# drtconway/zotmer

Hardware: AMD Instinct MI355X
Metric: Gk-mers/sec kmerize k=25 on synthetic 150bp FASTQ; achieved HBM GB/s fraction (higher is better)
Workload: dtype u64

## Files before the change

### zotmer_amd/csrc/context.hip

```cpp
#include <stdarg.h>
#include <string.h>

#include "internal.hpp"
#include <vector>

namespace zk {

int fail(zk_ctx* c, int code, const char* fmt, ...) {
    char buf[512];
    va_list ap;
    va_start(ap, fmt);
    vsnprintf(buf, sizeof buf, fmt, ap);
    va_end(ap);
    if (c) c->last_error = buf;
    return code;
}

void arena_reset(zk_ctx* c) { c->arena_off = 0; }

int arena_alloc(zk_ctx* c, uint64_t bytes, void** p) {
    const uint64_t need = (bytes + 255) & ~255ull;
    if (c->arena_off + need > c->arena_size) {
        if (c->arena_off != 0)
            return fail(c, ZK_ENOMEM, "workspace too small: %llu bytes in use, %llu more needed, %llu reserved (call zk_reserve)",
// ... 292 lines not shown
    if (what == ZK_TUNE_STREAM_PASS) {
#ifdef ZK_PHASES
        c->stream_pass = value < 0 ? 0 : value;
#else
        if (value < 0 || value > 3) return fail(c, ZK_EINVAL, "stream pass variant %d (0, 1, 2 or 3)", value);
        c->stream_pass = value;
#endif
        return ZK_OK;
    }
    if (what == ZK_TUNE_TAG_WORDS) { c->tag_words = value < 0 ? 0 : (value > 2 ? 2 : value); return ZK_OK; }
    if (what == ZK_TUNE_DEDUPE_VARIANT) { c->dedupe_variant = value < 0 ? -1 : (value & 3); return ZK_OK; }
    if (what == ZK_TUNE_KWAY) { c->kway = value < 0 ? 0 : (value > 2 ? 2 : value); return ZK_OK; }
    if (what == ZK_TUNE_TILE_SORT) { c->tile_sort = value ? 1 : 0; return ZK_OK; }
    if (what == ZK_TUNE_TAG_PASS) { c->tag_pass = value ? 1 : 0; return ZK_OK; }
    if (what == ZK_TUNE_DEDUPE_BITS) { c->dedupe_bits = value < 0 ? 0 : value; return ZK_OK; }
    if (what == ZK_TUNE_STRAND_BLOCKS) { c->strand_blocks = value < 0 ? 0 : (value > 3 ? 1 : value); return ZK_OK; }
    if (what == ZK_TUNE_DEDUPE_LIMIT) { c->dedupe_limit = value < 1 ? 1 : (value > 65536 ? 65536 : value); return ZK_OK; }
    if (what == ZK_TUNE_STREAM_RANGES) { c->stream_ranges = value < 0 ? 0 : (value > 4096 ? 4096 : value); return ZK_OK; }
    if (what == ZK_TUNE_XCD_GROUP) {
        if (value < 0 || value > 32 || (value & (value - 1))) return fail(c, ZK_EINVAL, "xcd group must be 0 or a power of two <= 32");
        c->xcd_group = value;
        return ZK_OK;
    }
    return fail(c, ZK_EINVAL, "unknown tuning knob %d", what);
}

int zk_debug_buffer(zk_ctx* c, void* d_buf) {
    if (!c) return ZK_EINVAL;
    enter(c);
    c->dbg = (u64*)d_buf;
    return ZK_OK;
// ... 99 lines not shown
```

### zotmer_amd/csrc/dedupe.hpp

```cpp
#pragma once
#include "internal.hpp"

namespace zk {

struct DedupeArgs {
    const u64* kin;
    const u32* tin;
    u64 n;
    const u64* cuts;
    u64* out;
    u64* nwords;
    int tag_bits;
    int pack;
    u32* flags;
    u32* counter;
    u64* big;
    u32* n_big;
    u32 big_cap;
    u32 chunks;
    u32* sub;
    u32* bad;
    u32* n_bad;
    u32 bad_cap;
    const u32* list;
    u32* retry;
    u32* n_retry;
    u32 limit;
    u64* dbg;
};

#ifdef ZK_PHASES
#define DD_PHASE(k) do { if (a.dbg) { const u32 now__ = (u32)__builtin_amdgcn_s_memtime(); ph[k] += now__ - tlast; tlast = now__; } } while (0)
#else
#define DD_PHASE(k) do { } while (0)
#endif

int launch_dedupe2(zk_ctx* c, const DedupeArgs& a, bool tagin, int variant, bool unsorted);

}
```

### zotmer_amd/csrc/dedupe2.hip

```cpp
#include "dedupe.hpp"
#include <type_traits>

namespace zk {

template <int BLOCK_, int BATCH_, int ITEMS_>
struct Dedupe2Smem {
    static constexpr int BLOCK = BLOCK_, BATCH = BATCH_, ITEMS = ITEMS_, TILE = BLOCK * ITEMS, NW = BLOCK / 64, ALL = 11264, SPT = ALL / BLOCK,
                         NB = 1024, SIDE = 64 + 64 * BATCH;
    static_assert(ALL % BLOCK == 0 && ALL % 8 == 0 && ITEMS % BATCH == 0 && ITEMS % 4 == 0, "whole rounds, whole quads, whole batches");
    alignas(16) u32 keys[ALL];
    alignas(16) u32 cnt[ALL / 2];
    union {
        u32 side[NW][SIDE];
        struct { u32 bc[NB]; u32 bbase[NB + 1]; } g;
    };
    u32 ticket;
    u32 nout;
};

template <int ITEMS>
struct Dedupe2Next {
    u32 chunk;
    u64 lo;
    u32 len;
    u32 tag[ITEMS];
};

template <int BLOCK, int ITEMS, bool TAGIN>
__device__ __forceinline__ void dedupe2_load(const DedupeArgs& a, u64 lo, u32 pos, u32 rem, u32 tmask, u32 (&t)[ITEMS]) {
    constexpr u32 TILE = BLOCK * ITEMS;
    u32 tid = threadIdx.x;
    asm volatile("" : "+v"(tid));
    if constexpr (TAGIN) {
// ... 11 lines not shown
            for (int i = 0; i < ITEMS; i++) {
                const u32 g = (u32)i * BLOCK + tid;
                t[i] = g < rem ? tp[g] : 0u;
            }
        }
    } else {
        const u64* kp = a.kin + lo + pos;
#pragma unroll
        for (int i = 0; i < ITEMS; i++) {
            const u32 g = (u32)i * BLOCK + tid;
            t[i] = g < rem ? (u32)kp[g] & tmask : 0u;
        }
    }
}

template <int BLOCK, int BATCH, int ITEMS_, bool TAGIN, bool UNSORTED>
__device__ __forceinline__ void dedupe2_block(const DedupeArgs& a, Dedupe2Smem<BLOCK, BATCH, ITEMS_>& sm, Dedupe2Next<ITEMS_>& st, u32 (&ph)[8], u32& tlast) {
    using S = Dedupe2Smem<BLOCK, BATCH, ITEMS_>;
    constexpr int ITEMS = S::ITEMS, TILE = S::TILE, ALL = S::ALL, SPT = S::SPT, NB = S::NB;
    constexpr u32 EMPTY = ~0u;
    constexpr u32 HS = ALL - 1;
    int tid = threadIdx.x;
    asm volatile("" : "+v"(tid));
    const int lane = tid & 63, wave = __builtin_amdgcn_readfirstlane(tid >> 6);
    const u32 chunk = st.chunk;
    const u64 lo = st.lo;
    const u32 len = st.len;
    const u32 maxc = (1u << a.pack) - 1u;
    const u32 tmask = a.tag_bits >= 32 ? ~0u : (1u << a.tag_bits) - 1u;
    auto next_block = [&](u32 t) {
        st.chunk = t; st.lo = 0; st.len = 0;
        if (t < a.chunks) {
            const u64 nlo = a.cuts[t], nhi = a.cuts[t + 1];
            st.lo = nlo;
// ... 76 lines not shown
    }
    drain(0, nside);
    DD_PHASE(1);
    const int any_bad = __syncthreads_or((int)bad);
    DD_PHASE(2);
    if (any_bad) {
        if (tid == 0) {
            a.retry[atomicAdd(a.n_retry, 1u)] = chunk;
            a.nwords[chunk] = 0;
        }
        if (a.sub && tid < 64) a.sub[(u64)chunk * 64 + tid] = 0;
        next_block(nchunk);
        return;
    }
    if constexpr (UNSORTED) {
        next_block(nchunk);
        const u16* cnt16 = reinterpret_cast<const u16*>(sm.cnt);
        u32 wn = 0;
#pragma unroll
        for (int j = 0; j < SPT; j++) wn += (u32)__popcll(__ballot(cnt16[tid + j * BLOCK] != 0));
        u32 wbase = 0;
        if (lane == 0 && wn) wbase = atomicAdd(&sm.nout, wn);
        wbase = (u32)__shfl((int)wbase, 0, 64);
        DD_PHASE(3);
        const u64 hi_part = (u64)chunk << a.tag_bits;
#pragma unroll
        for (int j = 0; j < SPT; j++) {
            const u32 c = cnt16[tid + j * BLOCK];
            const u64 bal = __ballot(c != 0);
            if (c) {
                const u64 k = hi_part | (u64)sm.keys[tid + j * BLOCK];
                if (c > maxc) {
                    const u32 at = atomicAdd(a.n_big, 1u);
                    if (at < a.big_cap) { a.big[2 * (u64)at] = k; a.big[2 * (u64)at + 1] = c; }
                    atomicOr(a.flags, 2u);
                }
                a.out[lo + wbase + popc_below(bal)] = (k << a.pack) | (u64)(c > maxc ? 0u : c);
            }
            wbase += (u32)__popcll(bal);
        }
        __syncthreads();
        if (tid == 0) a.nwords[chunk] = sm.nout;
        DD_PHASE(5);
        return;
    }
    for (int q = tid; q < NB; q += BLOCK) sm.g.bc[q] = 0;
    u32 et[SPT], ec[SPT];
    const int gb = a.tag_bits < 10 ? a.tag_bits : 10, bsh = a.tag_bits - gb;
    const u16* cnt16 = reinterpret_cast<const u16*>(sm.cnt);
#pragma unroll
    for (int j = 0; j < SPT; j++) {
        et[j] = sm.keys[tid + j * BLOCK];
        ec[j] = cnt16[tid + j * BLOCK];
    }
// ... 70 lines not shown
            const u32 i = i0 + e * BLOCK;
            if (i >= total) break;
            const u32 c = cc[e];
            const u64 k = hi_part | (u64)mine[e];
            if (c > maxc) {
                const u32 at = atomicAdd(a.n_big, 1u);
                if (at < a.big_cap) { a.big[2 * (u64)at] = k; a.big[2 * (u64)at + 1] = c; }
                atomicOr(a.flags, 2u);
            }
            a.out[lo + g0[e] + rank[e]] = (k << a.pack) | (u64)(c > maxc ? 0u : c);
        }
    }
    DD_PHASE(5);
}

template <int BLOCK, int BATCH, int ITEMS, bool TAGIN, bool UNSORTED>
__global__ __launch_bounds__(BLOCK, 2 * BLOCK / 256) void dedupe2_kernel(DedupeArgs a) {
    using S = Dedupe2Smem<BLOCK, BATCH, ITEMS>;
    __shared__ S sm;
    static_assert(sizeof(S) <= 80 * 1024, "two workgroups per CU");
    Dedupe2Next<ITEMS> st;
    if (threadIdx.x == 0) sm.ticket = atomicAdd(a.counter, 1u);
    __syncthreads();
    st.chunk = (u32)__builtin_amdgcn_readfirstlane((int)sm.ticket);
    st.lo = 0; st.len = 0;
    const u32 tmask = a.tag_bits >= 32 ? ~0u : (1u << a.tag_bits) - 1u;
    if (st.chunk < a.chunks) {
        const u64 nlo = a.cuts[st.chunk], nhi = a.cuts[st.chunk + 1];
        st.lo = nlo;
        st.len = nhi - nlo < (u64)a.limit ? (u32)(nhi - nlo) : ~0u;
    }
    if (st.len - 1u < ~0u - 1u) dedupe2_load<BLOCK, ITEMS, TAGIN>(a, st.lo, 0, st.len, tmask, st.tag);
    __syncthreads();
    u32 ph[8] = {0, 0, 0, 0, 0, 0, 0, 0};
    u32 tlast = a.dbg ? (u32)__builtin_amdgcn_s_memtime() : 0u;
    (void)tlast;
    u32 nblk = 0;
    while (st.chunk < a.chunks) {
        dedupe2_block<BLOCK, BATCH, ITEMS, TAGIN, UNSORTED>(a, sm, st, ph, tlast);
        __syncthreads();
        DD_PHASE(6);
        nblk++;
    }
    if (a.dbg && threadIdx.x == 0 && blockIdx.x < 256) {
        for (int k = 0; k < 8; k++) a.dbg[(u64)blockIdx.x * 16 + k] = ph[k];
        a.dbg[(u64)blockIdx.x * 16 + 8] = nblk;
    }
}

int launch_dedupe2(zk_ctx* c, const DedupeArgs& a, bool tagin, int variant, bool unsorted) {
    const u32 want = 2u * (u32)c->num_cus;
    const u32 grid = a.chunks < want ? a.chunks : want;
#define ZK_DD2(N, T, U) hipLaunchKernelGGL((dedupe2_kernel<512, N, 8, T, U>), dim3(grid), dim3(512), 0, c->stream, a)
#define ZK_DD2B(T, U) switch (variant & 3) { case 1: ZK_DD2(1, T, U); break; case 2: ZK_DD2(2, T, U); break; default: ZK_DD2(4, T, U); break; }
    if (unsorted) {
        if (tagin) ZK_DD2B(true, true) else ZK_DD2B(false, true)
    } else {
        if (tagin) ZK_DD2B(true, false) else ZK_DD2B(false, false)
    }
#undef ZK_DD2B
#undef ZK_DD2
    ZK_HIP(c, hipGetLastError());
    return ZK_OK;
}

}
```

### zotmer_amd/csrc/dedupe_blocks.hip

```cpp
#include "internal.hpp"
#include "dedupe.hpp"

namespace zk {

template <bool TAG32>
struct DedupeSmem {
    static constexpr int BLOCK = 1024, ITEMS = 8, TILE = BLOCK * ITEMS, NW = BLOCK / 64, ALL = TAG32 ? 12288 : 6144, SPT = ALL / BLOCK, NB = 256;
    static constexpr int SIDE_KEEP = 128, SIDE = SIDE_KEEP + 64 * ITEMS;
    typedef typename std::conditional<TAG32, u32, u64>::type E;
    E keys[ALL];
    u32 cnt[ALL];
    E side[NW][SIDE];
    u32 bc[NB];
    u32 bbase[NB + 1];
    u32 bfill[NB];
    u32 ticket;
};

__global__ void dedupe_cuts_kernel(const u64* __restrict__ k, u64 n, int tag_bits, u32 blocks, u64* __restrict__ cuts) {
    const u32 v = blockIdx.x * blockDim.x + threadIdx.x;
    if (v > blocks) return;
    u64 lo = 0, hi = n;
    while (lo < hi) {
        const u64 mid = (lo + hi) >> 1;
// ... 319 lines not shown
    }
}

int expand_tags(zk_ctx* c, const u32* tags, const u64* cuts, uint32_t blocks, int tag_bits, u64* keys_out, uint64_t first_block, uint64_t n_blocks) {
    if (n_blocks == 0) { first_block = 0; n_blocks = blocks; }
    hipLaunchKernelGGL(expand_tags_kernel, dim3(grid_cap(c, n_blocks, 16)), dim3(256), 0, c->stream, tags, cuts, (u64)first_block, (u64)n_blocks,
                       tag_bits, keys_out);
    ZK_HIP(c, hipGetLastError());
    return ZK_OK;
}

constexpr u32 DEDUPE_BIG_CAP = 1u << 16;
constexpr u32 DEDUPE_BAD_CAP = 64;

static int dedupe_lists(zk_ctx* c, const u64* keys, uint64_t n, int key_bits, int b, int pack, u64* work, uint64_t max_chunks,
                        const u32* tags, const u64* tag_cuts, bool unsorted, bool two_per_cu, DedupeArgs& a, DedupeResult* r) {
    uint64_t chunks = 1ull << b;
    if (max_chunks && chunks > max_chunks) chunks = max_chunks;
    u64 *cuts, *nwords, *incl, *big;
    if (tags) {
        if (!tag_cuts || key_bits - b > 32) return fail(c, ZK_EINTERNAL, "dedupe_pass: tags of %d bits", key_bits - b);
        cuts = const_cast<u64*>(tag_cuts);
    } else ZK_TRY(arena_alloc(c, sizeof(u64) * (chunks + 1), (void**)&cuts));
    ZK_TRY(arena_alloc(c, sizeof(u64) * chunks, (void**)&nwords));
    ZK_TRY(arena_alloc(c, sizeof(u64) * chunks, (void**)&incl));
    ZK_TRY(arena_alloc(c, sizeof(u64) * 2 * DEDUPE_BIG_CAP, (void**)&big));
    a.tag_bits = key_bits - b;
    if (!tags) hipLaunchKernelGGL(dedupe_cuts_kernel, dim3((u32)div_up(chunks + 1, 256)), dim3(256), 0, c->stream, keys, (u64)n, a.tag_bits, (u32)chunks, cuts);
    a.kin = keys; a.tin = tags; a.n = n; a.cuts = cuts; a.out = work; a.nwords = nwords; a.pack = pack;
    a.chunks = (u32)chunks;
    a.flags = (u32*)&c->d_scalars->dedupe_flags;
    a.counter = (u32*)&c->d_scalars->dedupe_counter;
    a.n_big = (u32*)&c->d_scalars->dedupe_n_big;
    a.big = big; a.big_cap = DEDUPE_BIG_CAP;
    ZK_TRY(arena_alloc(c, sizeof(u32) * DEDUPE_BAD_CAP, (void**)&a.bad));
    a.bad_cap = DEDUPE_BAD_CAP;
    a.n_bad = (u32*)&c->d_scalars->dedupe_n_bad;
    a.dbg = c->dbg ? c->dbg + 8192 : nullptr;
    unsorted = unsorted && two_per_cu;
    if (!max_chunks && !unsorted && a.tag_bits >= 14 && c->arena_size - c->arena_off > 64ull * chunks * (4 + 8 + 8) + (32ull << 20) + n / 16)
        ZK_TRY(arena_alloc(c, sizeof(u32) * 64 * chunks, (void**)&a.sub));
    ZK_HIP(c, hipMemsetAsync(&c->d_scalars->dedupe_flags, 0, ZK_SPAN(dedupe_flags, dedupe_n_bad), c->stream));
    r->cuts = cuts; r->nwords = nwords; r->incl = incl; r->big = big; r->chunks = (uint32_t)chunks; r->pack = pack; r->work = work;
    r->tag_bits = a.tag_bits; r->unsorted = unsorted;
    return ZK_OK;
}

static void launch_one_per_cu(zk_ctx* c, const DedupeArgs& d) {
    const u32 grid = d.chunks < (u32)c->num_cus ? d.chunks : (u32)c->num_cus;
    if (d.tin) hipLaunchKernelGGL((dedupe_kernel<true, true>), dim3(grid), dim3(1024), 0, c->stream, d);
    else if (d.tag_bits <= 32) hipLaunchKernelGGL((dedupe_kernel<true, false>), dim3(grid), dim3(1024), 0, c->stream, d);
    else hipLaunchKernelGGL((dedupe_kernel<false, false>), dim3(grid), dim3(1024), 0, c->stream, d);
}

static int dedupe_launch(zk_ctx* c, DedupeArgs& a, bool two_per_cu, bool unsorted) {
    prof_begin(c, ZK_PROF_RLE, (a.tin ? 4 : 8) * a.n);
    if (two_per_cu) {
        ZK_TRY(arena_alloc(c, sizeof(u32) * a.chunks, (void**)&a.retry));
        a.n_retry = (u32*)&c->d_scalars->dedupe_n_retry;
        a.limit = (u32)c->dedupe_limit;
        ZK_TRY(launch_dedupe2(c, a, a.tin != nullptr, c->dedupe_variant, unsorted));
    } else launch_one_per_cu(c, a);
    prof_end(c);
    ZK_HIP(c, hipGetLastError());
    ZK_TRY(fetch_span(c, &c->h_scalars->dedupe_flags, ZK_SPAN(dedupe_flags, dedupe_n_bad)));
    ZK_TRY(fetch(c, &c->h_scalars->dedupe_n_in, a.cuts + a.chunks));
    ZK_TRY(check_device_error(c));
    if (two_per_cu && (uint32_t)c->h_scalars->dedupe_n_retry) {
        DedupeArgs d = a;
        d.list = a.retry; d.chunks = (uint32_t)c->h_scalars->dedupe_n_retry; d.retry = nullptr; d.n_retry = nullptr;
        ZK_HIP(c, hipMemsetAsync(a.counter, 0, sizeof(u32), c->stream));
        launch_one_per_cu(c, d);
        ZK_HIP(c, hipGetLastError());
        ZK_TRY(fetch_span(c, &c->h_scalars->dedupe_flags, ZK_SPAN(dedupe_flags, dedupe_n_bad)));
        ZK_TRY(check_device_error(c));
    }
    return ZK_OK;
}

static int dedupe_bad_blocks(zk_ctx* c, const DedupeArgs& a, uint32_t n_bad, DedupeResult* r) {
    uint32_t list[DEDUPE_BAD_CAP];
    ZK_HIP(c, hipMemcpy(list, a.bad, sizeof(u32) * n_bad, hipMemcpyDeviceToHost));
    for (uint32_t i = 0; i < n_bad && !(r->flags & 1); i++) {
        u64 lohi[2];
        ZK_HIP(c, hipMemcpy(lohi, a.cuts + list[i], 2 * sizeof(u64), hipMemcpyDeviceToHost));
        const uint64_t m = lohi[1] - lohi[0];
        u64* res = nullptr;
        u64* bk = const_cast<u64*>(a.kin) + lohi[0];
        if (a.tin) {
            ZK_TRY(arena_alloc(c, 8 * m, (void**)&bk));
            ZK_TRY(expand_tags(c, a.tin, a.cuts, a.chunks, a.tag_bits, bk - lohi[0], list[i], 1));
        }
        ZK_TRY(sort_keys(c, bk, a.out + lohi[0], m, a.tag_bits, &res));
        if (res != bk) ZK_HIP(c, hipMemcpyAsync(bk, res, 8 * m, hipMemcpyDeviceToDevice, c->stream));
        uint64_t u = 0;
        bool ovf = false;
        ZK_TRY(rle(c, bk, m, a.out + lohi[0], nullptr, m, &u, a.pack, &ovf));
        if (ovf) { r->flags |= 1; break; }
        ZK_HIP(c, hipMemcpy(a.nwords + list[i], &u, sizeof(u64), hipMemcpyHostToDevice));
    }
    return ZK_OK;
}

int dedupe_pass(zk_ctx* c, const u64* keys, uint64_t n, int key_bits, int b, int pack, u64* work, uint64_t cap, DedupeResult* r,
                uint64_t* n_in, uint64_t max_chunks, const u32* tags, const u64* tag_cuts, bool unsorted) {
    *r = DedupeResult();
    if (n_in) *n_in = n;
    if (n == 0) return ZK_OK;
    if (b < 1 || b > 24 || b >= key_bits || pack < 10 || pack > 31) return fail(c, ZK_EINTERNAL, "dedupe_pass: %d block bits of %d, pack %d", b, key_bits, pack);
    if (cap < n) return fail(c, ZK_ENOSPC, "dedupe_pass: work buffer of %llu words for %llu keys", (unsigned long long)cap, (unsigned long long)n);
    DedupeArgs a = {};
    const bool two_per_cu = key_bits - b <= 32 && c->dedupe_variant >= 0;
    ZK_TRY(dedupe_lists(c, keys, n, key_bits, b, pack, work, max_chunks, tags, tag_cuts, unsorted, two_per_cu, a, r));
    ZK_TRY(dedupe_launch(c, a, two_per_cu, r->unsorted));
    r->flags = (uint32_t)c->h_scalars->dedupe_flags;
    r->n_big = (uint32_t)c->h_scalars->dedupe_n_big;
    if (r->n_big > DEDUPE_BIG_CAP) r->flags |= 1;
    const uint32_t n_bad = (uint32_t)c->h_scalars->dedupe_n_bad;
    if (n_bad && n_bad <= DEDUPE_BAD_CAP && !(r->flags & 1) && !max_chunks) {
        ZK_TRY(dedupe_bad_blocks(c, a, n_bad, r));
        a.sub = nullptr;
    } else if (n_bad > DEDUPE_BAD_CAP) r->flags |= 1;
    ZK_HIP(c, hipMemcpyAsync(r->incl, r->nwords, sizeof(u64) * r->chunks, hipMemcpyDeviceToDevice, c->stream));
    ZK_TRY(scan64_inclusive(c, r->incl, r->chunks));
    ZK_TRY(fetch(c, &c->h_scalars->dedupe_n_out, r->incl + r->chunks - 1));
    ZK_TRY(stream_sync(c));
    r->n_out = c->h_scalars->dedupe_n_out;
    prof_add_bytes(c, ZK_PROF_RLE, 8 * r->n_out);
    r->sub = a.sub;
// ... 52 lines not shown
```

### zotmer_amd/csrc/internal.hpp

```cpp
#pragma once
#include <hip/hip_runtime.h>
#include <stddef.h>
#include <stdint.h>
#include <stdio.h>
#include <string>
#include <vector>

#include "../../include/zotk.h"
#include "common.hpp"

struct zk_strand_counters { u32 n_declined, fail; };
struct zk_scalars {
    u64 rle_side;
    u64 total;
    u64 acgt[4];
    u64 n_keys;
    u64 rec_info[3];
    u64 sample_n;
    u64 dedupe_flags, dedupe_n_retry, dedupe_counter, dedupe_n_big, dedupe_n_bad;
    u64 dedupe_n_in;
    u64 dedupe_n_out;
    zk_strand_counters strand;
    u64 hist_big_n;
    u64 capture_kept;
    u64 capture_raw;
    u64 intersect_n;
    u64 checksum[3];
    u64 checksum_any[3];
    u64 stream_checksum[7];
    u64 first_descent;
    u64 ingest_cut;
    u64 sample_heads;
    u64 rle_overflow;
    u64 reduce_max;
// ... 13 lines not shown
    u64 vars[4];
    u64 links_bad;
    u64 render_bad;
    u64 render_bytes;
    u64 pileup_cursor;
    u64 pileup_long;
    u64 pulldown_vetoed;
    u64 capkmers_bad;
    u64 capkmers_total;
    u64 path_total;
    u64 place_bad;
    u64 place_slots;
    u64 seqtally[4];
};
#define ZK_SPAN(first, last) (offsetof(zk_scalars, last) + sizeof(zk_scalars::last) - offsetof(zk_scalars, first))
static_assert(sizeof(zk_scalars) == 81 * sizeof(u64), "zk_scalars: u64 words only, no padding");
static_assert(ZK_SPAN(rle_side, total) == 2 * sizeof(u64), "rle_prefix reads rle_side and total back as one range");
static_assert(ZK_SPAN(total, acgt) == 5 * sizeof(u64), "the merges read total and acgt back as one range");
static_assert(ZK_SPAN(acgt, n_keys) == 5 * sizeof(u64) && ZK_SPAN(acgt, sample_n) == 9 * sizeof(u64),
              "sort_stream reads acgt, n_keys, rec_info and sample_n back as one range");
static_assert(ZK_SPAN(rec_info, sample_n) == 4 * sizeof(u64), "sort_stream clears rec_info and sample_n as one range");
static_assert(offsetof(zk_scalars, dedupe_n_retry) == offsetof(zk_scalars, dedupe_flags) + 8 &&
              offsetof(zk_scalars, dedupe_counter) == offsetof(zk_scalars, dedupe_flags) + 16 &&
              offsetof(zk_scalars, dedupe_n_big) == offsetof(zk_scalars, dedupe_flags) + 24 &&
              ZK_SPAN(dedupe_flags, dedupe_n_bad) == 5 * sizeof(u64), "dedupe_pass clears and reads its five words as one range");

struct zk_ctx {
    int device = 0;
    hipStream_t stream = nullptr;
    bool own_stream = false;
    int num_cus = 256;
    int sort_variant = 3;
    int short_sort = 0;
    int packed_pairs = 1;
    int wide_tiles = 1;
    int early_collapse = 1;
    int side_div = 8;
    int pairs_variant = 7;
    int stream_pass = 1;
    int tag_words = 2;
// ... 112 lines not shown
int sort_pairs_mirrored(zk_ctx* c, const u64* src_k, const u32* src_v, u64* keys, u64* alt, u32* vals, u32* valt, uint64_t n, int K,
                        u64** rk, u32** rv, int lo_bit = 0);
int sort_pairs_rbits(zk_ctx* c);
struct StreamSample { int shift; uint64_t value; double max_ratio; uint64_t seen = 0, distinct = 0; bool want_distinct = false; };
struct StreamTags { bool written = false; u64* cuts = nullptr; uint32_t blocks = 0; };
struct StreamSrc { const u8* stream; uint64_t n_bytes; int K; int mode; int lo_bit; int hi_bit = 0; StreamSample* sample = nullptr;
                   StreamTags* tags = nullptr; };
int sort_stream(zk_ctx* c, const StreamSrc& src, u64* buf_a, u64* buf_b, uint64_t cap, uint64_t* n_keys,
                uint64_t acgt[4], u64** result);
int sort_rbits(zk_ctx* c);
PassPlan sort_plan_upper(zk_ctx* c, int key_bits, int lo_bit);
int sort_first_bits(zk_ctx* c, int key_bits, int lo_bit);
constexpr int MIRROR_RBITS = 9, MIRROR_RADIX = 1 << MIRROR_RBITS;
struct MirrorHist { int passes; int shift[4]; int bits[4]; u64* raw; };
int sort_keys_upper_counted(zk_ctx* c, u64* keys, u64* alt, uint64_t n, int key_bits, int lo_bit, u64* counted, u64** result);
struct DedupeResult {
    uint64_t n_out = 0;
    uint32_t flags = 0;
    uint32_t n_big = 0;
    u64 *cuts = nullptr, *nwords = nullptr, *incl = nullptr, *big = nullptr, *work = nullptr;
    u32* sub = nullptr;
    uint32_t chunks = 0;
    int pack = 0;
    int tag_bits = 0;
    bool unsorted = false;
};
int dedupe_pass(zk_ctx* c, const u64* keys, uint64_t n, int key_bits, int b, int pack, u64* work, uint64_t cap, DedupeResult* r,
                uint64_t* n_in = nullptr, uint64_t max_chunks = 0, const u32* tags = nullptr, const u64* tag_cuts = nullptr,
                bool unsorted = false);
int expand_tags(zk_ctx* c, const u32* tags, const u64* cuts, uint32_t blocks, int tag_bits, u64* keys_out, uint64_t first_block = 0, uint64_t n_blocks = 0);
int dedupe_finish(zk_ctx* c, const DedupeResult& r, u64* out_k, u32* out_c, u64* out_m = nullptr, int K = 0, int gbases = 0,
                  u64** mirror_hist = nullptr, int* mirror_group_bits = nullptr, bool packed_out = false);
int dedupe_sort_blocks(zk_ctx* c, DedupeResult& r);
int strand_blocks(zk_ctx* c, const DedupeResult& r, u64* keys_buf, uint64_t buf_words, int K, u64* out_k, u32* out_c, uint64_t cap,
                  uint64_t* n_out);
int collapse_pass(zk_ctx* c, const u64* keys, uint64_t n, int shift, int bits, int pack, u64* out, uint64_t cap, uint64_t* n_out,
                  uint64_t max_tiles = 0);
struct StreamRows { u32* rows = nullptr; u64* offs = nullptr; u32 ranges = 0, radix = 0; u32* gcodes = nullptr; u16* gvalid = nullptr;
                    u32 strands = 1;
                    bool wide = false; };
int stream_hist(zk_ctx* c, const u8* stream, uint64_t n_bytes, int K, int mode, const PassPlan& plan, u64* ghist, u32 gstride,
                u64* d_acgt, u64* d_n, u64* rec_info, u64* sample, u32 sample_cap, int sample_shift, u64 sample_value, u32* sample_n,
                void* image_room, uint64_t image_room_bytes, StreamRows* out);
struct StreamPlanes { u16* dig; int shift, bits; };
// ... 55 lines not shown
```

### zotmer_amd/csrc/pipeline.hip

```cpp
#include <string.h>

#include <vector>

#include "internal.hpp"

namespace zk {

__global__ void mirror_kernel(const u64* __restrict__ c, const u32* __restrict__ n, u64 m, int K, u64* __restrict__ r,
                              u32* __restrict__ v) {
    for (u64 i = (u64)blockIdx.x * blockDim.x + threadIdx.x; i < m; i += (u64)gridDim.x * blockDim.x) {
        r[i] = revcomp(K, c[i]);
        v[i] = n[i];
    }
}

constexpr int MIRROR_GROUP_BITS = 18;
constexpr int MIRROR_GROUP_BASES = MIRROR_GROUP_BITS / 2;

__global__ void mirror_bounds_kernel(const u64* __restrict__ c, u64 n, int K, int gbits, u64* __restrict__ start) {
    const u32 g = blockIdx.x * blockDim.x + threadIdx.x;
    if (g > (1u << gbits)) return;
    const u64 want = (u64)g << (2 * K - gbits);
    u64 lo = 0, hi = n;
    if (g == (1u << gbits)) lo = n;
// ... 260 lines not shown
        const int passes = lg > 15 ? (lg - 15 + rb - 1) / rb : 1;
        const int b = rb * passes;
        if (b < p.fused_bit + rb && b + rb / 2 < 2 * K && b <= 24 && (n_bytes >> b) >= 2048) p.dedupe_bit = b;
    }
    if (!both && c->early_collapse == 1 && c->dedupe_bits > 0 && p.pack && c->dedupe_bits % rb == 0 && c->dedupe_bits + rb / 2 < 2 * K &&
        c->dedupe_bits <= 24)
        p.dedupe_bit = c->dedupe_bits;
    p.tags = p.dedupe_bit && c->tag_words && 2 * K - p.dedupe_bit <= 32;
    p.tile_top = c->tile_sort ? tile_sort_top_bits(n_bytes, 2 * K, rb) : 0;
    p.both_top = tile_sort_top_bits(2 * n_bytes, 2 * K, rb);
    p.replan_pays = !canonical_only && c->tile_sort && p.both_top;
    p.look_bits = lg - 15 < 2 ? 2 : (lg - 15 > 30 ? 30 : lg - 15);
    p.look = !p.dedupe_bit && !both && c->early_collapse && !pack_bits_for(K) && p.tile_top && p.look_bits < 2 * K;
    p.blocks_mirror = !canonical_only && p.pack && p.dedupe_bit == MIRROR_GROUP_BITS && mirror_groups(K);
    p.blocks_strands = p.blocks_mirror && (K & 1) && c->strand_blocks;
    p.blocks_unsorted = p.blocks_mirror && (K & 1) && (c->strand_blocks == 1 || c->strand_blocks == 3);
    return p;
}

struct SortBufs {
    u64 *a, *b;
    uint64_t cap_keys;
    u64* other(const void* p) const { return p == a ? b : a; }
};
struct Output { u64* k; u32* c; uint64_t cap; uint64_t* n_out; };

struct Sorted {
    u64* keys = nullptr;
    u64* other = nullptr;
    uint64_t n = 0;
    StreamTags tags;
// ... 92 lines not shown
    if (p.canonical_only) ZK_TRY(tile_sort_count(c, s.keys, s.n, 2 * p.K, p.tile_top, o.k, o.c, o.cap, &r->uc, &declined));
    else ZK_TRY(tile_sort_count(c, s.keys, s.n, 2 * p.K, p.tile_top, s.keys, (u32*)s.other, s.n, &r->uc, &declined));
    if (declined) return count_by_passes(c, p, b, s.keys, s.n, 0, o, r);
    r->keys = s.keys; r->cnt = (u32*)s.other; r->where = p.canonical_only ? IN_OUTPUT : IN_SORT_BUF;
    return ZK_OK;
}

static int count_blocks(zk_ctx* c, const KmerizePlan& p, const SortBufs& b, const Sorted& s, const Output& o, zk_kmerize_stats* st, Counted* r) {
    const int K = p.K, pk = p.pack;
    DedupeResult d;
    uint64_t n_in = 0;
    const uint64_t nblocks = 1ull << p.dedupe_bit, per = s.n / nblocks + 1;
    const u32* tg = s.tags.written ? (const u32*)s.keys : nullptr;
    if (!s.presampled) ZK_TRY(dedupe_pass(c, s.keys, s.n, 2 * K, p.dedupe_bit, pk, s.other, b.cap_keys, &d, &n_in, (1u << 20) / per + 4, tg, s.tags.cuts));
    if (s.presampled || (!(d.flags & 1) && (double)d.n_out <= REPEAT_RATIO * (double)n_in)) {
        ZK_TRY(dedupe_pass(c, s.keys, s.n, 2 * K, p.dedupe_bit, pk, s.other, b.cap_keys, &d, nullptr, 0, tg, s.tags.cuts, p.blocks_unsorted));
        if (!(d.flags & 1)) {
            const uint64_t uc = r->uc = d.n_out;
            const bool want_m = !(d.flags & 2) && p.blocks_mirror;
            if (want_m && p.blocks_strands && 2 * align256(8 * uc) <= 8 * b.cap_keys) {
                st->n_canonical = uc;
                r->where = EMITTED;
                return strand_blocks(c, d, s.keys, b.cap_keys, K, o.k, o.c, o.cap, o.n_out);
            }
            if (d.unsorted) ZK_TRY(dedupe_sort_blocks(c, d));
            ZK_TRY(aux_list(c, uc, &r->keys, &r->cnt));
            ZK_TRY(dedupe_finish(c, d, r->keys, r->cnt, want_m ? s.keys : nullptr, K, MIRROR_GROUP_BASES, &r->mhist, &r->mgroup, want_m));
            if (want_m) { r->mwords = s.keys; r->malt = s.other; }
            r->where = IN_AUX;
            if (!(d.flags & 2)) { r->max_count = (1ull << pk) - 1; r->have_max = true; }
            return ZK_OK;
// ... 328 lines not shown
```

### zotmer_amd/csrc/strand_blocks.hip

```cpp
#include "tile_group.hpp"

namespace zk {

constexpr int SB_ITEMS = 16, SB_GROUPS = 2048;
constexpr u32 SB_GROUP_MAX = 128;
typedef TileSortSmem<SB_ITEMS, SB_GROUPS, false> StrandSmem;
constexpr int SB_BLOCK_BITS = 18;

__global__ __launch_bounds__(256) void strand_mirror_kernel(const u64* __restrict__ in, const u64* __restrict__ cuts, const u64* __restrict__ incl,
                                                            const u64* __restrict__ nwords, u32 chunks, int pack, int K, u64* __restrict__ out_m,
                                                            MirrorHist mh) {
    __shared__ u32 bins[4 * 512];
    const bool hist = mh.passes > 0;
    if (hist) {
        for (int q = threadIdx.x; q < 4 * 512; q += blockDim.x) bins[q] = 0;
        __syncthreads();
    }
    const u64 maxc = (1ull << pack) - 1;
    for (u32 v = blockIdx.x; v < chunks; v += gridDim.x) {
        const u64 cnt = nwords[v];
        const u64 dst0 = incl[v] - cnt;
        const u64* src = in + cuts[v];
        for (u64 i0 = threadIdx.x; i0 < cnt; i0 += 4ull * blockDim.x) {
            u64 w4[4];
#pragma unroll
            for (int q = 0; q < 4; q++) {
                const u64 i = i0 + (u64)q * blockDim.x;
                w4[q] = i < cnt ? src[i] : 0;
            }
#pragma unroll
            for (int q = 0; q < 4; q++) {
                const u64 i = i0 + (u64)q * blockDim.x;
                if (i >= cnt) break;
                const u64 mw = (revcomp(K, w4[q] >> pack) << pack) | (w4[q] & maxc);
                out_m[dst0 + i] = mw;
                if (hist) {
// ... 226 lines not shown
}

int strand_blocks(zk_ctx* c, const DedupeResult& r, u64* keys_buf, uint64_t buf_words, int K, u64* out_k, u32* out_c, uint64_t cap,
                  uint64_t* n_out) {
    *n_out = 0;
    const uint64_t uc = r.n_out;
    if (uc == 0) return ZK_OK;
    if (!(K & 1) || r.n_big || r.chunks != (1u << SB_BLOCK_BITS)) return fail(c, ZK_EINTERNAL, "strand_blocks: K %d, %u big counts, %u blocks", K, r.n_big, r.chunks);
    const uint64_t a8w = ((8 * uc + 255) & ~255ull) / 8;
    if (2 * a8w > buf_words) return fail(c, ZK_EINTERNAL, "strand_blocks: %llu words do not fit twice in %llu", (unsigned long long)uc, (unsigned long long)buf_words);
    if (2 * uc > cap) return fail(c, ZK_ENOSPC, "output holds %llu entries, the table has %llu", (unsigned long long)cap, (unsigned long long)(2 * uc));
    const int pk = r.pack, key_bits = 2 * K + pk, lo_bit = key_bits - SB_BLOCK_BITS;
    u64* mw = keys_buf;
    u64* malt = keys_buf + a8w;
    MirrorHist mh = {};
    if (c->sort_variant == 3) {
        const PassPlan plan = sort_plan_upper(c, key_bits, lo_bit);
        if (plan.passes <= 4) {
            ZK_TRY(arena_alloc(c, sizeof(u64) * MAX_PASSES * 512, (void**)&mh.raw));
            ZK_HIP(c, hipMemsetAsync(mh.raw, 0, sizeof(u64) * MAX_PASSES * 512, c->stream));
            mh.passes = plan.passes;
            for (int p = 0; p < plan.passes; p++) { mh.shift[p] = plan.shift[p]; mh.bits[p] = plan.bits[p]; }
        }
    }
    prof_begin(c, ZK_PROF_SELECT, 16 * uc);
    hipLaunchKernelGGL(strand_mirror_kernel, dim3((u32)c->num_cus * 8), dim3(256), 0, c->stream, r.work, r.cuts, r.incl, r.nwords, r.chunks, pk, K, mw, mh);
    prof_end(c);
    ZK_HIP(c, hipGetLastError());
    u64* sk = nullptr;
    if (mh.passes) ZK_TRY(sort_keys_upper_counted(c, mw, malt, uc, key_bits, lo_bit, mh.raw, &sk));
    else ZK_TRY(sort_keys_upper(c, mw, malt, uc, key_bits, lo_bit, &sk));
    u64* mstart;
    u32* declined;
    ZK_TRY(arena_alloc(c, sizeof(u64) * ((1ull << SB_BLOCK_BITS) + 1), (void**)&mstart));
    ZK_TRY(arena_alloc(c, sizeof(u32) * r.chunks, (void**)&declined));
    StrandArgs a = {};
    a.cw = r.work; a.cuts = r.cuts; a.nwords = r.nwords; a.incl = r.incl; a.m = sk; a.mstart = mstart;
    a.ok = out_k; a.oc = out_c; a.pack = pk; a.pshift = lo_bit;
    a.n_declined = &c->d_scalars->strand.n_declined;
    a.declined = declined;
    u32* fail = &c->d_scalars->strand.fail;
    prof_begin(c, ZK_PROF_UNION, 8 * 2 * uc + 12 * 2 * uc);
    hipLaunchKernelGGL(strand_starts_kernel, dim3(((1u << SB_BLOCK_BITS) + 256) / 256), dim3(256), 0, c->stream, sk, (u64)uc, lo_bit, mstart);
// ... 36 lines not shown
```

Baseline: 170.6.

## Fuse mirror-word emission and radix histogram into the unsorted dedupe kernel

The unsorted dedupe kernel now also writes the reverse-complement mirror words, placed through a global atomic cursor, into spare space in the keys buffer, and accumulates the upper-sort radix histograms in shared memory. strand_blocks then skips the separate strand_mirror_kernel pass, which re-read the deduped words. Chunks that went to the retry path are mirrored afterwards by a list-driven strand_mirror_kernel launch. The cost is extra shared-memory atomics and per-block syncs inside dedupe, one more host readback when there are retries, and new fallback logic when capacity or the sort plan does not match.

```diff
diff --git a/zotmer_amd/csrc/context.hip b/zotmer_amd/csrc/context.hip
--- a/zotmer_amd/csrc/context.hip
+++ b/zotmer_amd/csrc/context.hip
@@ -330,7 +330,7 @@
     if (what == ZK_TUNE_TILE_SORT) { c->tile_sort = value ? 1 : 0; return ZK_OK; }
     if (what == ZK_TUNE_TAG_PASS) { c->tag_pass = value ? 1 : 0; return ZK_OK; }
     if (what == ZK_TUNE_DEDUPE_BITS) { c->dedupe_bits = value < 0 ? 0 : value; return ZK_OK; }
-    if (what == ZK_TUNE_STRAND_BLOCKS) { c->strand_blocks = value < 0 ? 0 : (value > 3 ? 1 : value); return ZK_OK; }
+    if (what == ZK_TUNE_STRAND_BLOCKS) { c->strand_blocks = value < 0 ? 0 : (value > 5 ? 1 : value); return ZK_OK; }
     if (what == ZK_TUNE_DEDUPE_LIMIT) { c->dedupe_limit = value < 1 ? 1 : (value > 65536 ? 65536 : value); return ZK_OK; }
     if (what == ZK_TUNE_STREAM_RANGES) { c->stream_ranges = value < 0 ? 0 : (value > 4096 ? 4096 : value); return ZK_OK; }
     if (what == ZK_TUNE_XCD_GROUP) {
diff --git a/zotmer_amd/csrc/dedupe.hpp b/zotmer_amd/csrc/dedupe.hpp
--- a/zotmer_amd/csrc/dedupe.hpp
+++ b/zotmer_amd/csrc/dedupe.hpp
@@ -27,6 +27,11 @@
     u32* n_retry;
     u32 limit;
     u64* dbg;
+    u64* m_out;
+    u64* m_cursor;
+    u64 m_cap;
+    u64* m_hist;
+    int m_K, m_passes, m_shift[2], m_bits[2];
 };
 
 #ifdef ZK_PHASES
diff --git a/zotmer_amd/csrc/dedupe2.hip b/zotmer_amd/csrc/dedupe2.hip
--- a/zotmer_amd/csrc/dedupe2.hip
+++ b/zotmer_amd/csrc/dedupe2.hip
@@ -17,6 +17,11 @@
     u32 ticket;
     u32 nout;
 };
+template <int BLOCK_, int BATCH_, int ITEMS_>
+struct Dedupe2MirrorSmem : Dedupe2Smem<BLOCK_, BATCH_, ITEMS_> {
+    u32 bins[2][MIRROR_RADIX];
+    u64 mbase;
+};
 
 template <int ITEMS>
 struct Dedupe2Next {
@@ -58,10 +63,10 @@
     }
 }
 
-template <int BLOCK, int BATCH, int ITEMS_, bool TAGIN, bool UNSORTED>
-__device__ __forceinline__ void dedupe2_block(const DedupeArgs& a, Dedupe2Smem<BLOCK, BATCH, ITEMS_>& sm, Dedupe2Next<ITEMS_>& st, u32 (&ph)[8], u32& tlast) {
-    using S = Dedupe2Smem<BLOCK, BATCH, ITEMS_>;
-    constexpr int ITEMS = S::ITEMS, TILE = S::TILE, ALL = S::ALL, SPT = S::SPT, NB = S::NB;
+template <class S, bool TAGIN, bool UNSORTED, bool MIRROR>
+__device__ __forceinline__ void dedupe2_block(const DedupeArgs& a, S& sm, Dedupe2Next<S::ITEMS>& st, u32 (&ph)[8], u32& tlast) {
+    constexpr int BLOCK = S::BLOCK, BATCH = S::BATCH, ITEMS = S::ITEMS, TILE = S::TILE, ALL = S::ALL, SPT = S::SPT, NB = S::NB;
+    static_assert(!MIRROR || UNSORTED, "the mirror words are written beside the unsorted ones");
     constexpr u32 EMPTY = ~0u;
     constexpr u32 HS = ALL - 1;
     int tid = threadIdx.x;
@@ -168,7 +173,7 @@
         return;
     }
     if constexpr (UNSORTED) {
-        next_block(nchunk);
+        if constexpr (!MIRROR) next_block(nchunk);
         const u16* cnt16 = reinterpret_cast<const u16*>(sm.cnt);
         u32 wn = 0;
 #pragma unroll
@@ -176,6 +181,23 @@
         u32 wbase = 0;
         if (lane == 0 && wn) wbase = atomicAdd(&sm.nout, wn);
         wbase = (u32)__shfl((int)wbase, 0, 64);
+        u32 mrun = 0;
+        u64* mp = nullptr;
+        u64* op = nullptr;
+        if constexpr (MIRROR) {
+            __syncthreads();
+            u64 g = 0;
+            if (tid == 0) g = atomicAdd(a.m_cursor, (u64)sm.nout);
+            next_block(nchunk);
+            if (tid == 0) sm.mbase = g;
+            __syncthreads();
+            const u64 mb = sm.mbase;
+            const u64 mbase = ((u64)(u32)__builtin_amdgcn_readfirstlane((int)(mb >> 32)) << 32) | (u64)(u32)__builtin_amdgcn_readfirstlane((int)mb);
+            const u32 wb = (u32)__builtin_amdgcn_readfirstlane((int)wbase);
+            op = a.out + lo + wb;
+            if (mbase + sm.nout <= a.m_cap) mp = a.m_out + mbase + wb;
+            else if (tid == 0) atomicOr(a.flags, 4u);
+        }
         DD_PHASE(3);
         const u64 hi_part = (u64)chunk << a.tag_bits;
 #pragma unroll
@@ -189,9 +211,21 @@
                     if (at < a.big_cap) { a.big[2 * (u64)at] = k; a.big[2 * (u64)at + 1] = c; }
                     atomicOr(a.flags, 2u);
                 }
-                a.out[lo + wbase + popc_below(bal)] = (k << a.pack) | (u64)(c > maxc ? 0u : c);
-            }
-            wbase += (u32)__popcll(bal);
+                const u64 cw = (u64)(c > maxc ? 0u : c);
+                if constexpr (MIRROR) op[mrun + popc_below(bal)] = (k << a.pack) | cw;
+                else a.out[lo + wbase + popc_below(bal)] = (k << a.pack) | cw;
+                if constexpr (MIRROR) {
+                    if (mp) {
+                        const u64 mw = (revcomp(a.m_K, k) << a.pack) | cw;
+                        mp[mrun + popc_below(bal)] = mw;
+                        const u32 top = (u32)(mw >> a.m_shift[0]);
+                        atomicAdd(&sm.bins[0][top & ((1u << a.m_bits[0]) - 1u)], 1u);
+                        atomicAdd(&sm.bins[1][(top >> a.m_bits[0]) & (MIRROR_RADIX - 1)], 1u);
+                    }
+                }
+            }
+            if constexpr (MIRROR) mrun += (u32)__popcll(bal);
+            else wbase += (u32)__popcll(bal);
         }
         __syncthreads();
         if (tid == 0) a.nwords[chunk] = sm.nout;
@@ -292,12 +326,14 @@
     DD_PHASE(5);
 }
 
-template <int BLOCK, int BATCH, int ITEMS, bool TAGIN, bool UNSORTED>
+template <int BLOCK, int BATCH, int ITEMS, bool TAGIN, bool UNSORTED, bool MIRROR = false>
 __global__ __launch_bounds__(BLOCK, 2 * BLOCK / 256) void dedupe2_kernel(DedupeArgs a) {
-    using S = Dedupe2Smem<BLOCK, BATCH, ITEMS>;
+    using S = typename std::conditional<MIRROR, Dedupe2MirrorSmem<BLOCK, BATCH, ITEMS>, Dedupe2Smem<BLOCK, BATCH, ITEMS>>::type;
     __shared__ S sm;
     static_assert(sizeof(S) <= 80 * 1024, "two workgroups per CU");
     Dedupe2Next<ITEMS> st;
+    if constexpr (MIRROR)
+        for (int q = threadIdx.x; q < 2 * MIRROR_RADIX; q += BLOCK) (&sm.bins[0][0])[q] = 0;
     if (threadIdx.x == 0) sm.ticket = atomicAdd(a.counter, 1u);
     __syncthreads();
     st.chunk = (u32)__builtin_amdgcn_readfirstlane((int)sm.ticket);
@@ -315,11 +351,17 @@
     (void)tlast;
     u32 nblk = 0;
     while (st.chunk < a.chunks) {
-        dedupe2_block<BLOCK, BATCH, ITEMS, TAGIN, UNSORTED>(a, sm, st, ph, tlast);
+        dedupe2_block<S, TAGIN, UNSORTED, MIRROR>(a, sm, st, ph, tlast);
         __syncthreads();
         DD_PHASE(6);
         nblk++;
     }
+    if constexpr (MIRROR) {
+        for (int q = threadIdx.x; q < a.m_passes * MIRROR_RADIX; q += BLOCK) {
+            const u32 x = (&sm.bins[0][0])[q];
+            if (x) atomicAdd(&a.m_hist[q], (u64)x);
+        }
+    }
     if (a.dbg && threadIdx.x == 0 && blockIdx.x < 256) {
         for (int k = 0; k < 8; k++) a.dbg[(u64)blockIdx.x * 16 + k] = ph[k];
         a.dbg[(u64)blockIdx.x * 16 + 8] = nblk;
@@ -329,6 +371,14 @@
 int launch_dedupe2(zk_ctx* c, const DedupeArgs& a, bool tagin, int variant, bool unsorted) {
     const u32 want = 2u * (u32)c->num_cus;
     const u32 grid = a.chunks < want ? a.chunks : want;
+    if (a.m_out) {
+        if (!tagin || !unsorted || !a.m_cursor || !a.m_hist || a.m_passes < 1 || a.m_passes > 2 || a.m_bits[0] > MIRROR_RBITS || a.m_bits[1] > MIRROR_RBITS)
+            return fail(c, ZK_EINTERNAL, "launch_dedupe2: mirror words with %d passes, tags %d, unsorted %d", a.m_passes, (int)tagin, (int)unsorted);
+        if ((variant & 3) == 1) hipLaunchKernelGGL((dedupe2_kernel<512, 1, 8, true, true, true>), dim3(grid), dim3(512), 0, c->stream, a);
+        else hipLaunchKernelGGL((dedupe2_kernel<512, 2, 8, true, true, true>), dim3(grid), dim3(512), 0, c->stream, a);
+        ZK_HIP(c, hipGetLastError());
+        return ZK_OK;
+    }
 #define ZK_DD2(N, T, U) hipLaunchKernelGGL((dedupe2_kernel<512, N, 8, T, U>), dim3(grid), dim3(512), 0, c->stream, a)
 #define ZK_DD2B(T, U) switch (variant & 3) { case 1: ZK_DD2(1, T, U); break; case 2: ZK_DD2(2, T, U); break; default: ZK_DD2(4, T, U); break; }
     if (unsorted) {
diff --git a/zotmer_amd/csrc/dedupe_blocks.hip b/zotmer_amd/csrc/dedupe_blocks.hip
--- a/zotmer_amd/csrc/dedupe_blocks.hip
+++ b/zotmer_amd/csrc/dedupe_blocks.hip
@@ -357,7 +357,7 @@
 constexpr u32 DEDUPE_BAD_CAP = 64;
 
 static int dedupe_lists(zk_ctx* c, const u64* keys, uint64_t n, int key_bits, int b, int pack, u64* work, uint64_t max_chunks,
-                        const u32* tags, const u64* tag_cuts, bool unsorted, bool two_per_cu, DedupeArgs& a, DedupeResult* r) {
+                        const u32* tags, const u64* tag_cuts, bool unsorted, bool two_per_cu, const DedupeMirror* mirror, DedupeArgs& a, DedupeResult* r) {
     uint64_t chunks = 1ull << b;
     if (max_chunks && chunks > max_chunks) chunks = max_chunks;
     u64 *cuts, *nwords, *incl, *big;
@@ -383,7 +383,19 @@
     unsorted = unsorted && two_per_cu;
     if (!max_chunks && !unsorted && a.tag_bits >= 14 && c->arena_size - c->arena_off > 64ull * chunks * (4 + 8 + 8) + (32ull << 20) + n / 16)
         ZK_TRY(arena_alloc(c, sizeof(u32) * 64 * chunks, (void**)&a.sub));
-    ZK_HIP(c, hipMemsetAsync(&c->d_scalars->dedupe_flags, 0, ZK_SPAN(dedupe_flags, dedupe_n_bad), c->stream));
+    if (mirror && mirror->out && mirror->cap && unsorted && tags && !max_chunks && c->sort_variant == 3) {
+        const PassPlan plan = sort_plan_upper(c, key_bits + pack, key_bits + pack - b);
+        if (plan.passes <= 2) {
+            ZK_TRY(arena_alloc(c, sizeof(u64) * MAX_PASSES * MIRROR_RADIX, (void**)&a.m_hist));
+            ZK_HIP(c, hipMemsetAsync(a.m_hist, 0, sizeof(u64) * MAX_PASSES * MIRROR_RADIX, c->stream));
+            a.m_out = mirror->out; a.m_cap = mirror->cap; a.m_K = mirror->K; a.m_passes = plan.passes;
+            a.m_cursor = &c->d_scalars->dedupe_m_cursor;
+            r->mh.passes = plan.passes; r->mh.raw = a.m_hist;
+            for (int p = 0; p < plan.passes; p++) { a.m_shift[p] = r->mh.shift[p] = plan.shift[p]; a.m_bits[p] = r->mh.bits[p] = plan.bits[p]; }
+            r->m_words = a.m_out; r->m_cap = a.m_cap;
+        }
+    }
+    ZK_HIP(c, hipMemsetAsync(&c->d_scalars->dedupe_flags, 0, ZK_SPAN(dedupe_flags, dedupe_m_cursor), c->stream));
     r->cuts = cuts; r->nwords = nwords; r->incl = incl; r->big = big; r->chunks = (uint32_t)chunks; r->pack = pack; r->work = work;
     r->tag_bits = a.tag_bits; r->unsorted = unsorted;
     return ZK_OK;
@@ -396,7 +408,7 @@
     else hipLaunchKernelGGL((dedupe_kernel<false, false>), dim3(grid), dim3(1024), 0, c->stream, d);
 }
 
-static int dedupe_launch(zk_ctx* c, DedupeArgs& a, bool two_per_cu, bool unsorted) {
+static int dedupe_launch(zk_ctx* c, DedupeArgs& a, bool two_per_cu, bool unsorted, DedupeResult* r) {
     prof_begin(c, ZK_PROF_RLE, (a.tin ? 4 : 8) * a.n);
     if (two_per_cu) {
         ZK_TRY(arena_alloc(c, sizeof(u32) * a.chunks, (void**)&a.retry));
@@ -406,16 +418,21 @@
     } else launch_one_per_cu(c, a);
     prof_end(c);
     ZK_HIP(c, hipGetLastError());
-    ZK_TRY(fetch_span(c, &c->h_scalars->dedupe_flags, ZK_SPAN(dedupe_flags, dedupe_n_bad)));
+    ZK_TRY(fetch_span(c, &c->h_scalars->dedupe_flags, ZK_SPAN(dedupe_flags, dedupe_m_cursor)));
     ZK_TRY(fetch(c, &c->h_scalars->dedupe_n_in, a.cuts + a.chunks));
     ZK_TRY(check_device_error(c));
+    if (two_per_cu) { r->retry = a.retry; r->n_retry = (uint32_t)c->h_scalars->dedupe_n_retry; }
+    if (a.m_out) {
+        r->m_placed = c->h_scalars->dedupe_m_cursor;
+        r->m_emitted = !((uint32_t)c->h_scalars->dedupe_flags & 4u) && r->m_placed <= a.m_cap;
+    }
     if (two_per_cu && (uint32_t)c->h_scalars->dedupe_n_retry) {
         DedupeArgs d = a;
         d.list = a.retry; d.chunks = (uint32_t)c->h_scalars->dedupe_n_retry; d.retry = nullptr; d.n_retry = nullptr;
         ZK_HIP(c, hipMemsetAsync(a.counter, 0, sizeof(u32), c->stream));
         launch_one_per_cu(c, d);
         ZK_HIP(c, hipGetLastError());
-        ZK_TRY(fetch_span(c, &c->h_scalars->dedupe_flags, ZK_SPAN(dedupe_flags, dedupe_n_bad)));
+        ZK_TRY(fetch_span(c, &c->h_scalars->dedupe_flags, ZK_SPAN(dedupe_flags, dedupe_m_cursor)));
         ZK_TRY(check_device_error(c));
     }
     return ZK_OK;
@@ -446,7 +463,7 @@
 }
 
 int dedupe_pass(zk_ctx* c, const u64* keys, uint64_t n, int key_bits, int b, int pack, u64* work, uint64_t cap, DedupeResult* r,
-                uint64_t* n_in, uint64_t max_chunks, const u32* tags, const u64* tag_cuts, bool unsorted) {
+                uint64_t* n_in, uint64_t max_chunks, const u32* tags, const u64* tag_cuts, bool unsorted, const DedupeMirror* mirror) {
     *r = DedupeResult();
     if (n_in) *n_in = n;
     if (n == 0) return ZK_OK;
@@ -454,8 +471,8 @@
     if (cap < n) return fail(c, ZK_ENOSPC, "dedupe_pass: work buffer of %llu words for %llu keys", (unsigned long long)cap, (unsigned long long)n);
     DedupeArgs a = {};
     const bool two_per_cu = key_bits - b <= 32 && c->dedupe_variant >= 0;
-    ZK_TRY(dedupe_lists(c, keys, n, key_bits, b, pack, work, max_chunks, tags, tag_cuts, unsorted, two_per_cu, a, r));
-    ZK_TRY(dedupe_launch(c, a, two_per_cu, r->unsorted));
+    ZK_TRY(dedupe_lists(c, keys, n, key_bits, b, pack, work, max_chunks, tags, tag_cuts, unsorted, two_per_cu, mirror, a, r));
+    ZK_TRY(dedupe_launch(c, a, two_per_cu, r->unsorted, r));
     r->flags = (uint32_t)c->h_scalars->dedupe_flags;
     r->n_big = (uint32_t)c->h_scalars->dedupe_n_big;
     if (r->n_big > DEDUPE_BIG_CAP) r->flags |= 1;
diff --git a/zotmer_amd/csrc/internal.hpp b/zotmer_amd/csrc/internal.hpp
--- a/zotmer_amd/csrc/internal.hpp
+++ b/zotmer_amd/csrc/internal.hpp
@@ -18,6 +18,7 @@
     u64 rec_info[3];
     u64 sample_n;
     u64 dedupe_flags, dedupe_n_retry, dedupe_counter, dedupe_n_big, dedupe_n_bad;
+    u64 dedupe_m_cursor;
     u64 dedupe_n_in;
     u64 dedupe_n_out;
     zk_strand_counters strand;
@@ -61,7 +62,7 @@
     u64 seqtally[4];
 };
 #define ZK_SPAN(first, last) (offsetof(zk_scalars, last) + sizeof(zk_scalars::last) - offsetof(zk_scalars, first))
-static_assert(sizeof(zk_scalars) == 81 * sizeof(u64), "zk_scalars: u64 words only, no padding");
+static_assert(sizeof(zk_scalars) == 82 * sizeof(u64), "zk_scalars: u64 words only, no padding");
 static_assert(ZK_SPAN(rle_side, total) == 2 * sizeof(u64), "rle_prefix reads rle_side and total back as one range");
 static_assert(ZK_SPAN(total, acgt) == 5 * sizeof(u64), "the merges read total and acgt back as one range");
 static_assert(ZK_SPAN(acgt, n_keys) == 5 * sizeof(u64) && ZK_SPAN(acgt, sample_n) == 9 * sizeof(u64),
@@ -70,7 +71,7 @@
 static_assert(offsetof(zk_scalars, dedupe_n_retry) == offsetof(zk_scalars, dedupe_flags) + 8 &&
               offsetof(zk_scalars, dedupe_counter) == offsetof(zk_scalars, dedupe_flags) + 16 &&
               offsetof(zk_scalars, dedupe_n_big) == offsetof(zk_scalars, dedupe_flags) + 24 &&
-              ZK_SPAN(dedupe_flags, dedupe_n_bad) == 5 * sizeof(u64), "dedupe_pass clears and reads its five words as one range");
+              ZK_SPAN(dedupe_flags, dedupe_m_cursor) == 6 * sizeof(u64), "dedupe_pass clears and reads its six words as one range");
 
 struct zk_ctx {
     int device = 0;
@@ -213,6 +214,7 @@
 constexpr int MIRROR_RBITS = 9, MIRROR_RADIX = 1 << MIRROR_RBITS;
 struct MirrorHist { int passes; int shift[4]; int bits[4]; u64* raw; };
 int sort_keys_upper_counted(zk_ctx* c, u64* keys, u64* alt, uint64_t n, int key_bits, int lo_bit, u64* counted, u64** result);
+struct DedupeMirror { u64* out = nullptr; uint64_t cap = 0; int K = 0; };
 struct DedupeResult {
     uint64_t n_out = 0;
     uint32_t flags = 0;
@@ -223,10 +225,16 @@
     int pack = 0;
     int tag_bits = 0;
     bool unsorted = false;
+    bool m_emitted = false;
+    u64* m_words = nullptr;
+    uint64_t m_cap = 0, m_placed = 0;
+    MirrorHist mh = {};
+    u32* retry = nullptr;
+    uint32_t n_retry = 0;
 };
 int dedupe_pass(zk_ctx* c, const u64* keys, uint64_t n, int key_bits, int b, int pack, u64* work, uint64_t cap, DedupeResult* r,
                 uint64_t* n_in = nullptr, uint64_t max_chunks = 0, const u32* tags = nullptr, const u64* tag_cuts = nullptr,
-                bool unsorted = false);
+                bool unsorted = false, const DedupeMirror* mirror = nullptr);
 int expand_tags(zk_ctx* c, const u32* tags, const u64* cuts, uint32_t blocks, int tag_bits, u64* keys_out, uint64_t first_block = 0, uint64_t n_blocks = 0);
 int dedupe_finish(zk_ctx* c, const DedupeResult& r, u64* out_k, u32* out_c, u64* out_m = nullptr, int K = 0, int gbases = 0,
                   u64** mirror_hist = nullptr, int* mirror_group_bits = nullptr, bool packed_out = false);
diff --git a/zotmer_amd/csrc/pipeline.hip b/zotmer_amd/csrc/pipeline.hip
--- a/zotmer_amd/csrc/pipeline.hip
+++ b/zotmer_amd/csrc/pipeline.hip
@@ -298,7 +298,7 @@
     p.look = !p.dedupe_bit && !both && c->early_collapse && !pack_bits_for(K) && p.tile_top && p.look_bits < 2 * K;
     p.blocks_mirror = !canonical_only && p.pack && p.dedupe_bit == MIRROR_GROUP_BITS && mirror_groups(K);
     p.blocks_strands = p.blocks_mirror && (K & 1) && c->strand_blocks;
-    p.blocks_unsorted = p.blocks_mirror && (K & 1) && (c->strand_blocks == 1 || c->strand_blocks == 3);
+    p.blocks_unsorted = p.blocks_mirror && (K & 1) && (c->strand_blocks == 1 || c->strand_blocks >= 3);
     return p;
 }
 
@@ -421,7 +421,13 @@
     const u32* tg = s.tags.written ? (const u32*)s.keys : nullptr;
     if (!s.presampled) ZK_TRY(dedupe_pass(c, s.keys, s.n, 2 * K, p.dedupe_bit, pk, s.other, b.cap_keys, &d, &n_in, (1u << 20) / per + 4, tg, s.tags.cuts));
     if (s.presampled || (!(d.flags & 1) && (double)d.n_out <= REPEAT_RATIO * (double)n_in)) {
-        ZK_TRY(dedupe_pass(c, s.keys, s.n, 2 * K, p.dedupe_bit, pk, s.other, b.cap_keys, &d, nullptr, 0, tg, s.tags.cuts, p.blocks_unsorted));
+        DedupeMirror mo;
+        const uint64_t tag_words = align256(4 * s.n) / 8;
+        if (tg && p.blocks_strands && p.blocks_unsorted && c->strand_blocks != 4 && tag_words < b.cap_keys) {
+            mo.out = s.keys + tag_words; mo.cap = b.cap_keys - tag_words; mo.K = K;
+            if (c->strand_blocks == 5 && mo.cap > 1024) mo.cap = 1024;
+        }
+        ZK_TRY(dedupe_pass(c, s.keys, s.n, 2 * K, p.dedupe_bit, pk, s.other, b.cap_keys, &d, nullptr, 0, tg, s.tags.cuts, p.blocks_unsorted, &mo));
         if (!(d.flags & 1)) {
             const uint64_t uc = r->uc = d.n_out;
             const bool want_m = !(d.flags & 2) && p.blocks_mirror;
diff --git a/zotmer_amd/csrc/strand_blocks.hip b/zotmer_amd/csrc/strand_blocks.hip
--- a/zotmer_amd/csrc/strand_blocks.hip
+++ b/zotmer_amd/csrc/strand_blocks.hip
@@ -9,17 +9,26 @@
 
 __global__ __launch_bounds__(256) void strand_mirror_kernel(const u64* __restrict__ in, const u64* __restrict__ cuts, const u64* __restrict__ incl,
                                                             const u64* __restrict__ nwords, u32 chunks, int pack, int K, u64* __restrict__ out_m,
-                                                            MirrorHist mh) {
+                                                            MirrorHist mh, const u32* __restrict__ list, u64* cursor, u64 m_cap) {
     __shared__ u32 bins[4 * 512];
+    __shared__ u64 placed;
     const bool hist = mh.passes > 0;
     if (hist) {
         for (int q = threadIdx.x; q < 4 * 512; q += blockDim.x) bins[q] = 0;
         __syncthreads();
     }
     const u64 maxc = (1ull << pack) - 1;
-    for (u32 v = blockIdx.x; v < chunks; v += gridDim.x) {
+    for (u32 t = blockIdx.x; t < chunks; t += gridDim.x) {
+        const u32 v = list ? list[t] : t;
         const u64 cnt = nwords[v];
-        const u64 dst0 = incl[v] - cnt;
+        u64 dst0 = incl[v] - cnt;
+        if (list) {
+            if (threadIdx.x == 0) placed = atomicAdd(cursor, cnt);
+            __syncthreads();
+            dst0 = placed;
+            __syncthreads();
+            if (dst0 + cnt > m_cap) continue;
+        }
         const u64* src = in + cuts[v];
         for (u64 i0 = threadIdx.x; i0 < cnt; i0 += 4ull * blockDim.x) {
             u64 w4[4];
@@ -276,19 +285,48 @@
     u64* mw = keys_buf;
     u64* malt = keys_buf + a8w;
     MirrorHist mh = {};
-    if (c->sort_variant == 3) {
+    bool fused = r.m_emitted && r.m_words >= keys_buf && r.m_words + r.m_cap <= keys_buf + buf_words && uc <= r.m_cap && c->sort_variant == 3;
+    if (fused) {
         const PassPlan plan = sort_plan_upper(c, key_bits, lo_bit);
-        if (plan.passes <= 4) {
-            ZK_TRY(arena_alloc(c, sizeof(u64) * MAX_PASSES * 512, (void**)&mh.raw));
-            ZK_HIP(c, hipMemsetAsync(mh.raw, 0, sizeof(u64) * MAX_PASSES * 512, c->stream));
-            mh.passes = plan.passes;
-            for (int p = 0; p < plan.passes; p++) { mh.shift[p] = plan.shift[p]; mh.bits[p] = plan.bits[p]; }
-        }
-    }
-    prof_begin(c, ZK_PROF_SELECT, 16 * uc);
-    hipLaunchKernelGGL(strand_mirror_kernel, dim3((u32)c->num_cus * 8), dim3(256), 0, c->stream, r.work, r.cuts, r.incl, r.nwords, r.chunks, pk, K, mw, mh);
-    prof_end(c);
-    ZK_HIP(c, hipGetLastError());
+        fused = plan.passes == r.mh.passes;
+        for (int p = 0; fused && p < plan.passes; p++) fused = plan.shift[p] == r.mh.shift[p] && plan.bits[p] == r.mh.bits[p];
+        const uint64_t before = (uint64_t)(r.m_words - keys_buf), behind = buf_words - before;
+        if (before < a8w && behind < 2 * a8w) fused = false;
+        if (fused) malt = before >= a8w ? keys_buf : r.m_words + a8w;
+    }
+    if (fused) {
+        mw = r.m_words;
+        mh = r.mh;
+        uint64_t placed = r.m_placed;
+        prof_begin(c, ZK_PROF_SELECT, 16 * uc);
+        if (r.n_retry) {
+            hipLaunchKernelGGL(strand_mirror_kernel, dim3(grid_cap(c, r.n_retry, 8)), dim3(256), 0, c->stream, r.work, r.cuts, r.incl, r.nwords, r.n_retry, pk, K,
+                               mw, mh, r.retry, &c->d_scalars->dedupe_m_cursor, (u64)r.m_cap);
+        }
+        prof_end(c);
+        if (r.n_retry) {
+            ZK_HIP(c, hipGetLastError());
+            ZK_TRY(fetch(c, &c->h_scalars->dedupe_m_cursor));
+            ZK_TRY(stream_sync(c));
+            placed = c->h_scalars->dedupe_m_cursor;
+        }
+        if (placed != uc) return fail(c, ZK_EINTERNAL, "strand_blocks: %llu mirror words for %llu entries", (unsigned long long)placed, (unsigned long long)uc);
+    } else {
+        if (c->sort_variant == 3) {
+            const PassPlan plan = sort_plan_upper(c, key_bits, lo_bit);
+            if (plan.passes <= 4) {
+                ZK_TRY(arena_alloc(c, sizeof(u64) * MAX_PASSES * 512, (void**)&mh.raw));
+                ZK_HIP(c, hipMemsetAsync(mh.raw, 0, sizeof(u64) * MAX_PASSES * 512, c->stream));
+                mh.passes = plan.passes;
+                for (int p = 0; p < plan.passes; p++) { mh.shift[p] = plan.shift[p]; mh.bits[p] = plan.bits[p]; }
+            }
+        }
+        prof_begin(c, ZK_PROF_SELECT, 16 * uc);
+        hipLaunchKernelGGL(strand_mirror_kernel, dim3((u32)c->num_cus * 8), dim3(256), 0, c->stream, r.work, r.cuts, r.incl, r.nwords, r.chunks, pk, K, mw, mh,
+                           (const u32*)nullptr, (u64*)nullptr, (u64)0);
+        prof_end(c);
+        ZK_HIP(c, hipGetLastError());
+    }
     u64* sk = nullptr;
     if (mh.passes) ZK_TRY(sort_keys_upper_counted(c, mw, malt, uc, key_bits, lo_bit, mh.raw, &sk));
     else ZK_TRY(sort_keys_upper(c, mw, malt, uc, key_bits, lo_bit, &sk));
```

New measurement: 173.6 (median of 6 runs). 1.02x the previous value.
